# LUOJIUzxy/PortfolioOptGP

Hardware: AMD Instinct MI355X
Metric: GP fits/sec (N=4096, 1-D RBF) (higher is better)
Workload: dtype f64

## Files before the change

portfoliooptgp_amd/csrc/gpx_band16.hip:

```cpp
#include <hip/hip_runtime.h>
#include <hip/hip_ext.h>
#include "gpx_internal.h"
#include "gpx_leaf.h"
#include "gpx_b16core.h"

namespace gpx {


#ifdef GPX_BAND_PHASES
__device__ unsigned long long g_b16_phase[2][16];
#define Q_BEGIN unsigned long long qp_t = __builtin_amdgcn_s_memtime(), qp_acc[12] = {};
#define QP(i)                                                        \
  do {                                                               \
    const unsigned long long qp_n = __builtin_amdgcn_s_memtime();    \
    qp_acc[i] += qp_n - qp_t;                                        \
    qp_t = qp_n;                                                     \
  } while (0)
#define Q_END(kid)                                                                 \
  do {                                                                             \
    if (threadIdx.x == 0) {                                                        \
      for (int qp_i = 0; qp_i < 12; ++qp_i) atomicAdd(&g_b16_phase[kid][qp_i], qp_acc[qp_i]); \
      atomicAdd(&g_b16_phase[kid][15], 1ull);                                      \
    }                                                                              \
  } while (0)
#else
#define Q_BEGIN
#define QP(i) \
  do {        \
  } while (0)
#define Q_END(kid) \
  do {             \
  } while (0)
#endif

namespace {

__device__ __forceinline__ t4 ktile_t(const double* __restrict__ K, long long ld, int bi, int bj, int l15, int l4,
                                      int kband) {
  t4 t;
  const int gi = bi * 16 + l15;
#pragma unroll
  for (int r = 0; r < 4; ++r) {
    const int gj = bj * 16 + 4 * r + l4;
    const int i0 = max(gi, gj), j0 = min(gi, gj);
    const bool z = (i0 >> 6) - (j0 >> 6) >= kband;
    const double v = K[(long long)i0 * ld + (z ? i0 : j0)];
    t[r] = z ? 0.0 : v;
  }
  return t;
}

constexpr __host__ __device__ int wid(int i, int j) { return i * (i + 1) / 2 + j; }

__device__ __forceinline__ void exp4(const double (&x)[4], double (&e)[4]) {
  constexpr double c[13] = {0x1.71547652b82fep+0, -0x1.62e42fefa39efp-1, -0x1.abc9e3b39803fp-56,
                            0x1.ade156a5dcb37p-26, 0x1.28af3fca7ab0cp-22, 0x1.71dee623fde64p-19,
                            0x1.a01997c89e6b0p-16, 0x1.a01a014761f6ep-13, 0x1.6c16c1852b7b0p-10,
                            0x1.1111111122322p-7, 0x1.55555555502a1p-5, 0x1.5555555555511p-3,
                            0x1.000000000000bp-1};
  double k[4], r[4], p[4];
#pragma unroll
  for (int q = 0; q < 4; ++q) {
    k[q] = __builtin_rint(x[q] * c[0]);
    r[q] = __builtin_fma(k[q], c[1], x[q]);
  }
#pragma unroll
  for (int q = 0; q < 4; ++q) r[q] = __builtin_fma(k[q], c[2], r[q]);
#pragma unroll
  for (int q = 0; q < 4; ++q) p[q] = __builtin_fma(r[q], c[3], c[4]);
#pragma unroll
  for (int i = 5; i <= 12; ++i)
#pragma unroll
    for (int q = 0; q < 4; ++q) p[q] = __builtin_fma(r[q], p[q], c[i]);
#pragma unroll
  for (int q = 0; q < 4; ++q) {
    p[q] = __builtin_fma(r[q], p[q], 1.0);
    p[q] = __builtin_fma(r[q], p[q], 1.0);
    const double v = __builtin_amdgcn_ldexp(p[q], (int)k[q]);
    e[q] = !(x[q] < -1075.0) ? v : 0.0;
  }
}
struct ExpLib {
  __device__ __forceinline__ void load() {}
  __device__ __forceinline__ double exp(double x) const { return ::exp(x); }
  __device__ __forceinline__ void exp4(const double (&x)[4], double (&e)[4]) const { gpx::exp4(x, e); }
};

template <class EXP>
__device__ __forceinline__ double k_se1(double m2ai, double ai2, double aj, bool ok, bool diag, double var,
                                       double noise, const EXP& E) {
  if (!ok) return diag ? 1.0 : 0.0;
  const double v = var * E.exp(-0.5 * sqdist1_b(aj, m2ai, ai2));
  return diag ? v + noise : v;
}
__device__ __forceinline__ void ktile_store(double* __restrict__ K, long long ld, int bi, int bj, const t4& t, int l15,
                                            int l4) {
  double* p = K + (long long)(bi * 16 + l15) * ld + bj * 16 + l4;
#pragma unroll
  for (int r = 0; r < 4; ++r) p[4 * r] = t[r];
}
__device__ __forceinline__ int rq(int il) { return (il & 3) * 4 + (il >> 2); }

}

#ifndef GPX_B16_FWD3_WAVES
#define GPX_B16_FWD3_WAVES 2
#endif
template <int Q, bool KIN>
struct Fwd16 {
  static constexpr int kNew = 16 * kSC, kXa = kNew + (KIN ? 1 : Q + 1) * 256, size = kXa + (KIN ? Q + 1 : 1) * 16;
};
template <int Q, bool KIN>
__device__ __forceinline__ void fwd_sweep(const BandFusedArgs& a, double* __restrict__ lds) {
  double* sc = lds;
  double(*snew)[256] = reinterpret_cast<double(*)[256]>(lds + Fwd16<Q, KIN>::kNew);
  double(*sxa)[16] = reinterpret_cast<double(*)[16]>(lds + Fwd16<Q, KIN>::kXa);
  const unsigned long long wt0 = a.wtrace ? __builtin_amdgcn_s_memrealtime() : 0ull;
  const int b = a.active[blockIdx.x];
  const int Np = a.Np, nb = Np >> 4;
  const long long ld = a.ld;
  double* K = a.K + (long long)b * a.sMat;
  double* L = a.L + (long long)b * a.sMat;
  double* z = a.z + (long long)b * a.sVec;
  double* ldiag = a.ldiag + (long long)b * a.sVec;
  const bool kst = KIN && a.kstore;
  const double* y = a.Y + (long long)b * a.sY;
  const int n = a.nvalid[b];
  const int lane = threadIdx.x, l15 = lane & 15, l4 = lane >> 4;
  constexpr int NW = (Q + 1) * (Q + 2) / 2;
  const double* X = a.X + (long long)b * a.sX;
  int xd0 = 0;
  double kell = 1.0, kvar = 1.0, knoise = 0.0;
  ExpLib E;
  if constexpr (KIN) {
    E.load();
    const gpx_term& tm = a.specs[b].terms[0];
    const double* th = a.theta + (long long)b * GPX_THETA_STRIDE;
    xd0 = tm.dim_start;
    kell = th[tm.param_offset];
    kvar = th[tm.param_offset + 1];
    knoise = th[a.specs[b].n_params];
  }
  const int D = a.D;
  auto xval = [&](int g) { return X[(long long)min(g, n - 1) * D + xd0]; };
  t4 T[NW];
  double u[Q + 1];
  if constexpr (KIN) {
    if (l4 == 0) {
#pragma unroll
      for (int m = 0; m <= Q; ++m) sxa[m][rq(l15)] = m < nb ? xval(m * 16 + l15) / kell : 0.0;
    }
    wsync();
#pragma unroll
    for (int i = 0; i <= Q; ++i) {
      u[i] = 0.0;
      const double ar = i < nb ? xval(i * 16 + l15) / kell : 0.0;
      const int gi = i * 16 + l15;
#pragma unroll
      for (int j = 0; j <= i; ++j) {
        t4 t = tzero();
        if (i < nb) {
          const t4 ac = *reinterpret_cast<const t4*>(&sxa[j][4 * l4]);
#pragma unroll
          for (int r = 0; r < 4; ++r) {
            const int gj = j * 16 + 4 * r + l4;
            const bool zero = (gi >> 6) - (gj >> 6) >= a.kband;
            t[r] = zero ? 0.0 : k_se1(-2.0 * ar, ar * ar, ac[r], gi < n && gj < n, gi == gj, kvar, knoise, E);
          }
          if (kst) ktile_store(K, ld, i, j, t, l15, l4);
        }
        T[wid(i, j)] = t;
      }
    }
  } else {
#pragma unroll
    for (int i = 0; i <= Q; ++i) {
      u[i] = 0.0;
#pragma unroll
      for (int j = 0; j <= i; ++j) T[wid(i, j)] = (i < nb) ? ktile_t(K, ld, i, j, l15, l4, a.kband) : tzero();
    }
  }
  int gfail = 0;
  Q_BEGIN
  auto step = [&](const int k, const auto qkc, const auto fullc) __attribute__((always_inline)) {
    const int qk = qkc, k16 = k * 16;
    const int bn = k + Q + 1;
    const bool newrow = decltype(fullc)::value || bn < nb;
    double xn = 0.0;
    if constexpr (KIN) {
      if (newrow) xn = xval(bn * 16 + l15);
    } else {
      wsync();
      lds_drain();
      if (newrow) {
#pragma unroll
        for (int j = 0; j <= Q; ++j) tile_glds_swz(K + (long long)(bn * 16) * ld + (k + 1 + j) * 16, ld, snew[j], lane);
      }
    }
    double yl = y[min(k16 + l15, n - 1)];
    yl = k16 + l15 < n ? yl : 0.0;
    QP(0);
    t4 V;
    double lii;
    int fl;
    double* Lk = L + (long long)k * ((Q + 1) * 256);
    double zr[4];
    {
      t4 Wr;
      leaf16m(T[wid(0, 0)], V, Wr, lii, fl, sc, l15, l4);
      frag_store(Wr, Lk, lane);
      QP(1);
      const double yu = yl + u[0];
#pragma unroll
      for (int r = 0; r < 4; ++r) zr[r] = sum16(Wr[r] * yu);
    }
    if (fl >= 0 && gfail == 0) gfail = k16 + fl + 1;
    QP(2);
#pragma unroll
    for (int i = 1; i <= Q; ++i) {
      if (i <= qk) {
        t4 c = tzero();
        mma(c, V, T[wid(i, 0)]);
        T[wid(i, 0)] = c;
        double s = 0.0;
#pragma unroll
        for (int r = 0; r < 4; ++r) s = fma(c[r], zr[r], s);
        u[i] -= sum4(s);
      }
    }
    QP(3);
#pragma unroll
    for (int i = 1; i <= Q; ++i)
#pragma unroll
      for (int j = 1; j <= i; ++j)
        if (i <= qk) mms(T[wid(i, j)], T[wid(j, 0)], T[wid(i, 0)]);
    QP(4);
    vm_drain();
    wsync();
    QP(6);
#pragma unroll
    for (int i = 1; i <= Q; ++i)
      if (i <= qk) frag_store(T[wid(i, 0)], Lk + i * 256, lane);
    if (l4 == 0) ldiag[k16 + l15] = lii;
    if (l15 == 0) {
#pragma unroll
      for (int r = 0; r < 4; ++r) z[k16 + 4 * r + l4] = zr[r];
    }
#pragma unroll
    for (int i = 0; i < Q; ++i) {
#pragma unroll
      for (int j = 0; j <= i; ++j) T[wid(i, j)] = T[wid(i + 1, j + 1)];
      u[i] = u[i + 1];
    }
    u[Q] = 0.0;
    QP(7);
    if constexpr (KIN) {
      const double ar = xn / kell, m2ar = -2.0 * ar, ar2 = ar * ar;
      if (newrow && l4 == 0) sxa[bn % (Q + 1)][rq(l15)] = ar;
      wsync();
      const int gi = bn * 16 + l15;
#pragma unroll
      for (int j = 0; j <= Q; ++j) {
        t4 t = tzero();
        const int c = k + 1 + j;
        if (newrow && (bn >> 2) - (c >> 2) < a.kband) {
          const t4 ac = *reinterpret_cast<const t4*>(&sxa[c % (Q + 1)][4 * l4]);
          double xe[4], ev[4];
#pragma unroll
          for (int r = 0; r < 4; ++r) xe[r] = -0.5 * sqdist1_b(ac[r], m2ar, ar2);
          E.exp4(xe, ev);
          if (bn * 16 + 16 <= n) {
#pragma unroll
            for (int r = 0; r < 4; ++r) {
              const double v = kvar * ev[r];
              t[r] = (j == Q && 4 * r + l4 == l15) ? v + knoise : v;
            }
          } else {
#pragma unroll
            for (int r = 0; r < 4; ++r) {
              const int gj = c * 16 + 4 * r + l4;
              const double v = kvar * ev[r];
              t[r] = !(gi < n && gj < n) ? (gi == gj ? 1.0 : 0.0) : (gi == gj ? v + knoise : v);
            }
          }
          if (kst) ktile_store(K, ld, bn, c, t, l15, l4);
        }
        T[wid(Q, j)] = t;
      }
    } else {
#pragma unroll
      for (int j = 0; j <= Q; ++j) {
        t4 t = tzero();
        if (newrow) {
          const bool zero = (bn >> 2) - ((k + 1 + j) >> 2) >= a.kband;
#pragma unroll
          for (int r = 0; r < 4; ++r) {
            const int cl = 4 * r + l4;
            const double v = (j == Q && cl > l15) ? snew[j][swz16(cl, l15)] : snew[j][swz16(l15, cl)];
            t[r] = zero ? 0.0 : v;
          }
        }
        T[wid(Q, j)] = t;
      }
    }
    QP(5);
  };
  int k = 0;
  if constexpr (Q != 4)
    for (; k < nb - Q - 1; ++k) step(k, std::integral_constant<int, Q>{}, std::true_type{});
  for (; k < nb; ++k) step(k, min(Q, nb - 1 - k), std::false_type{});
  Q_END(0);
  if (lane == 0 && gfail > 0 && a.info[b] == 0) a.info[b] = gfail;
  wave_trace_put(a, wt0, Q);
}

template <int Q, bool KIN>
__global__ __launch_bounds__(64, Q <= 3 ? GPX_B16_FWD3_WAVES : (Q <= 4 ? 2 : 1)) void band16_fwd_kernel(BandFusedArgs a) {
  __shared__ __attribute__((aligned(16))) double lds[Fwd16<Q, KIN>::size];
  fwd_sweep<Q, KIN>(a, lds);
}

#ifndef GPX_B16_BWD_2W_QMAX
#define GPX_B16_BWD_2W_QMAX 3
#endif
template <int Q, int NT, bool SE1, bool KIN>
struct Bwd16 {
  static constexpr int kZ = 16 * kSC;
  static constexpr int nZ = SE1 ? (KIN ? 0 : 2 * (Q + 1)) : Q + 1;
  static constexpr int kAl = kZ + nZ * 256;
  static constexpr int kAlT = kAl + (SE1 ? 0 : (Q + 1) * 16);
  static constexpr int kXT = kAlT + (SE1 ? (Q + 1) * 16 : 0);
  static constexpr int kCs = kXT + (SE1 ? (Q + 1) * 16 : 0);
  static constexpr int kTh = kCs + (Q + 1) * 16;
  static constexpr int kRed = kTh + (SE1 ? 0 : 16);
  static constexpr bool LP = SE1 && KIN && Q == 4;
  static constexpr int kPf = kRed + (SE1 ? 0 : 16);
  static constexpr int size = kPf + (LP ? (Q + 1) * 256 : 0);
};
template <int Q, int NT, bool SE1, bool KIN>
__device__ __forceinline__ void bwd_sweep(const BandFusedArgs& a, double* __restrict__ lds, double* __restrict__ sx) {
  static_assert(!SE1 || KIN || Q <= 5, "the SE1 sweep double-buffers its K tiles in LDS: Q <= 5");
  static_assert(!KIN || SE1, "inline K tiles: SE1 sweeps only");
  using Ly = Bwd16<Q, NT, SE1, KIN>;
  double* sc = lds;
  double(*sz)[256] = reinterpret_cast<double(*)[256]>(lds + Ly::kZ);
  double(*sal)[16] = reinterpret_cast<double(*)[16]>(lds + Ly::kAl);
  double(*salT)[16] = reinterpret_cast<double(*)[16]>(lds + Ly::kAlT);
  double(*sxT)[16] = reinterpret_cast<double(*)[16]>(lds + Ly::kXT);
  double(*scs)[16] = reinterpret_cast<double(*)[16]>(lds + Ly::kCs);
  double* sth = SE1 ? lds : lds + Ly::kTh;
  double* sred = SE1 ? lds + 16 : lds + Ly::kRed;
  const unsigned long long wt0 = a.wtrace ? __builtin_amdgcn_s_memrealtime() : 0ull;
  const int b = a.active[blockIdx.x];
  const int Np = a.Np, nb = Np >> 4;
  const long long ld = a.ld;
  double* Kd = a.K + (long long)b * a.sMat;
  const double* L = a.L + (long long)b * a.sMat;
  const double* z = a.z + (long long)b * a.sVec;
  double* alpha = a.alpha + (long long)b * a.sVec;
  const double* X = a.X + (long long)b * a.sX;
  const int n = a.nvalid[b], D = a.D, nx = 16 * D;
  const int lane = threadIdx.x, l15 = lane & 15, l4 = lane >> 4;
  auto fetch = [&](int kk, double (&zr)[4], double (&xr)[2]) {
    const int q1 = min(Q, nb - 1 - kk), c16 = kk * 16;
    if constexpr (SE1 && !KIN) {
#pragma unroll
      for (int i = 0; i <= Q; ++i)
        if (i <= q1) tile_glds_swz(Kd + (long long)(c16 + 16 * i) * ld + c16, ld, sz[(kk & 1) * (Q + 1) + i], lane);
    }
#pragma unroll
    for (int r = 0; r < 4; ++r) zr[r] = z[c16 + 4 * r + l4];
#pragma unroll
    for (int h = 0; h < 2; ++h) {
      const int e = lane + 64 * h;
      xr[h] = X[min((long long)c16 * D + e, (long long)n * D - 1)];
    }
  };
  constexpr bool LP = Ly::LP;
  double* spf = lds + Ly::kPf;
  auto fetch_f = [&](int kk, t4& Wn, t4 (&Pn)[Q + 1]) {
    const int q1 = min(Q, nb - 1 - kk);
    const double* Lk = L + (long long)kk * ((Q + 1) * 256) + 4 * lane;
    if constexpr (LP) {
#pragma unroll
      for (int i = 0; i <= Q; ++i)
        if (i <= q1) {
          __builtin_amdgcn_global_load_lds(Lk + i * 256, spf + i * 256, 16, 0, 0);
          __builtin_amdgcn_global_load_lds(Lk + i * 256 + 2, spf + i * 256 + 128, 16, 0, 0);
        }
    } else {
      Wn = *reinterpret_cast<const t4*>(Lk);
#pragma unroll
      for (int i = 1; i <= Q; ++i) Pn[i] = (i <= q1) ? *reinterpret_cast<const t4*>(Lk + i * 256) : tzero();
    }
  };
  auto lds_tile = [&](int i) {
    const double2 a0 = *reinterpret_cast<const double2*>(spf + i * 256 + 2 * lane);
    const double2 a1 = *reinterpret_cast<const double2*>(spf + i * 256 + 128 + 2 * lane);
    return (t4){a0.x, a0.y, a1.x, a1.y};
  };
  double zr[4], xr[2];
  t4 Wn, Pn[Q + 1];
  fetch(nb - 1, zr, xr);
  fetch_f(nb - 1, Wn, Pn);
  {
    double* ldg = a.ldiag + (long long)b * a.sVec;
    for (int e = lane; e < Np; e += 64) ldg[e] = log(ldg[e]);
  }
  if (lane < GPX_THETA_STRIDE) sth[lane] = a.theta[b * GPX_THETA_STRIDE + lane];
  if (lane < 16) {
#pragma unroll
    for (int m = 0; m <= Q; ++m) {
      scs[m][lane] = 0.0;
      if constexpr (SE1) {
        salT[m][lane] = 0.0;
        sxT[m][lane] = 0.0;
      } else {
        sal[m][lane] = 0.0;
      }
    }
  }
  vm_drain();
  wsync();
  const DevSpec spec = a.specs[b];
  const int fkind = spec.terms[0].kind, fd0 = spec.terms[0].dim_start, fdn = spec.terms[0].dim_count;
  const bool fast = (NT == 1) && spec.n_terms == 1 && fkind >= GPX_SE && fkind <= GPX_EXPONENTIAL;
  const double fvar = sth[spec.terms[0].param_offset + 1];
  const double finv_ell = 1.0 / sth[spec.terms[0].param_offset];
  const double xscale = fast ? sth[spec.terms[0].param_offset] : 1.0;
  const double noise = sth[spec.n_params];
  double sums[NT][3];
#pragma unroll
  for (int t = 0; t < NT; ++t) sums[t][0] = sums[t][1] = sums[t][2] = 0.0;
  double snoise = 0.0, resmax = 0.0;
  constexpr int NS = Q * (Q + 1) / 2;
  t4 S[NS];
#pragma unroll
  for (int e = 0; e < NS; ++e) S[e] = tzero();
  double al[Q + 1];
  t4 R[Q + 1];
#pragma unroll
  for (int i = 0; i <= Q; ++i) {
    al[i] = 0.0;
    R[i] = tzero();
  }
  Q_BEGIN
  for (int k = nb - 1; k >= 0; --k) {
    const int qk = min(Q, nb - 1 - k), k16 = k * 16, cs = k % (Q + 1);
    t4 Wf, P[Q + 1];
    if constexpr (LP) {
      vm_drain();
      wsync();
      Wf = lds_tile(0);
#pragma unroll
      for (int i = 1; i <= Q; ++i) P[i] = (i <= qk) ? lds_tile(i) : tzero();
    } else {
      Wf = Wn;
#pragma unroll
      for (int i = 1; i <= Q; ++i) P[i] = Pn[i];
    }
    if constexpr (!SE1) {
#pragma unroll
      for (int h = 0; h < 2; ++h) {
        const int e = lane + 64 * h;
        if (e < nx) sx[cs * nx + e] = (k16 + e / D < n) ? xr[h] / xscale : 0.0;
      }
      for (int e = lane + 128; e < nx; e += 64) sx[cs * nx + e] = (k16 + e / D < n) ? X[(long long)k16 * D + e] / xscale : 0.0;
    } else {
#pragma unroll
      for (int h = 0; h < 2; ++h) {
        const int e = lane + 64 * h, il = e / D;
        if (e < nx && e - il * D == fd0) sxT[cs][(il & 3) * 4 + (il >> 2)] = (k16 + il < n) ? xr[h] / xscale : 0.0;
      }
    }
    const double zc[4] = {zr[0], zr[1], zr[2], zr[3]};
    lds_drain();
    wsync();
    if (k > 0) fetch(k - 1, zr, xr);
    QP(0);
    double t[4] = {0.0, 0.0, 0.0, 0.0};
#pragma unroll
    for (int i = 1; i <= Q; ++i) {
      double ai;
      if constexpr (LP)
        ai = salT[(k + i) % (Q + 1)][(l15 & 3) * 4 + (l15 >> 2)];
      else
        ai = al[i];
#pragma unroll
      for (int r = 0; r < 4; ++r) t[r] = fma(P[i][r], ai, t[r]);
    }
    double ap = 0.0;
#pragma unroll
    for (int r = 0; r < 4; ++r) ap = fma(Wf[r], zc[r] - sum16(t[r]), ap);
    ap = sum4(ap);
    al[0] = ap;
    if (l4 == 0) {
      if constexpr (SE1)
        salT[cs][(l15 & 3) * 4 + (l15 >> 2)] = ap;
      else
        sal[cs][l15] = ap;
    }
    QP(1);
#pragma unroll
    for (int i = 1; i <= Q; ++i) {
      t4 g = tzero();
      mma(g, P[i], Wf);
      P[i] = g;
    }
    QP(2);
    t4 Zn[Q + 1];
#pragma unroll
    for (int i = 1; i <= Q; ++i) {
      Zn[i] = tzero();
#pragma unroll
      for (int j = 1; j <= Q; ++j) {
        if (j >= i) {
          mms(Zn[i], S[wid(j - 1, i - 1)], P[j]);
        } else {
          const t4 tt = tile_transpose(S[wid(i - 1, j - 1)], sc, l15, l4);
          mms(Zn[i], tt, P[j]);
        }
      }
    }
    QP(3);
    if (k > 0) fetch_f(k - 1, Wn, Pn);
    t4 Zk = tzero();
    mma(Zk, Wf, Wf);
#pragma unroll
    for (int i = 1; i <= Q; ++i) mms(Zk, P[i], Zn[i]);
    wsync();
    QP(4);
    const int gj = k16 + l15;
    const bool jok = gj < n;
    const double* xj = sx + cs * nx + l15 * D;
    double colacc = 0.0;
    if constexpr (SE1) {
      const double xjv = sxT[cs][(l15 & 3) * 4 + (l15 >> 2)];
      const double m2xj = -2.0 * xjv, xj2 = xjv * xjv;
#pragma unroll
      for (int i = 0; i <= Q; ++i) {
        if (i > qk) continue;
        const t4& Zt = (i == 0) ? Zk : Zn[i];
        const int si = (k + i) % (Q + 1);
        const double w = i == 0 ? 1.0 : 2.0;
        const t4 a4 = *reinterpret_cast<const t4*>(&salT[si][4 * l4]);
        const t4 x4 = *reinterpret_cast<const t4*>(&sxT[si][4 * l4]);
        const bool zero = ((k + i) >> 2) - (k >> 2) >= a.kband;
        double r2v[4], kexp[4] = {0.0, 0.0, 0.0, 0.0};
#pragma unroll
        for (int r = 0; r < 4; ++r) r2v[r] = sqdist1_b(x4[r], m2xj, xj2);
        if constexpr (KIN) {
          if (!zero) {
            double xe[4];
#pragma unroll
            for (int r = 0; r < 4; ++r) xe[r] = -0.5 * r2v[r];
            exp4(xe, kexp);
          }
        }
#pragma unroll
        for (int r = 0; r < 4; ++r) {
          const int il = 4 * r + l4, gi = (k + i) * 16 + il;
          const double zij = Zt[r];
          const double ai = a4[r];
          const double r2 = r2v[r];
          const bool dg = i == 0 && il == l15;
          double kraw;
          if constexpr (KIN) {
            kraw = 0.0;
            if (!zero) {
              const double kv = fvar * kexp[r];
              kraw = dg ? kv + noise : kv;
            }
          } else {
            const bool up = i == 0 && il < l15;
            kraw = sz[(k & 1) * (Q + 1) + i][up ? swz16(l15, il) : swz16(il, l15)];
          }
          const double v = w * fma(ai, ap, -zij);
          const bool ok = i > 0 || (jok && gi < n);
          const double kij = KIN ? (ok ? kraw : 0.0) : ((zero || !ok) ? 0.0 : kraw);
          const double kg = i > 0 ? kij : (ok ? (dg ? fvar : kij) : 0.0);
          sums[0][0] = fma(v, kg * r2, sums[0][0]);
          sums[0][1] = fma(v, kg, sums[0][1]);
          snoise = (ok && dg) ? snoise + v : snoise;
          const double kz = kij * zij;
          colacc += kz;
          if (i > 0) R[i][r] += kz;
        }
      }
    } else {
#pragma unroll
      for (int i = 0; i <= Q; ++i)
        if (i <= qk) {
          const t4& Zt = (i == 0) ? Zk : Zn[i];
#pragma unroll
          for (int r = 0; r < 4; ++r) sz[i][(4 * r + l4) * 16 + l15] = Zt[r];
        }
      wsync();
      double rowp[Q + 1][4];
#pragma unroll
      for (int i = 0; i <= Q; ++i)
#pragma unroll
        for (int r = 0; r < 4; ++r) rowp[i][r] = 0.0;
      for (int i = 0; i <= qk; ++i) {
        const int si = (k + i) % (Q + 1);
        const double w = i == 0 ? 1.0 : 2.0;
#pragma unroll
        for (int r = 0; r < 4; ++r) {
          const int il = 4 * r + l4, gi = (k + i) * 16 + il;
          const double zij = sz[i][il * 16 + l15];
          const double ai = sal[si][il];
          const double* xi = sx + si * nx + il * D;
          const bool ok = jok && gi < n;
          const bool dg = i == 0 && gi == gj;
          const double v = w * fma(ai, ap, -zij);
          double kij = 0.0;
          if (ok) {
            double dk[NT][3];
            if (fast) {
              double d1[3];
              stationary_grad(fkind, sqdist_scaled(xi + fd0, xj + fd0, fdn), fvar, finv_ell, d1);
              dk[0][0] = d1[0]; dk[0][1] = d1[1]; dk[0][2] = d1[2];
              kij = fvar * d1[1];
            } else {
              kij = eval_k_grad<NT>(spec, sth, xi, xj, dk);
            }
#pragma unroll
            for (int q = 0; q < NT; ++q) {
              sums[q][0] = fma(v, dk[q][0], sums[q][0]);
              sums[q][1] = fma(v, dk[q][1], sums[q][1]);
              sums[q][2] = fma(v, dk[q][2], sums[q][2]);
            }
          }
          if (dg) kij += noise;
          snoise = (ok && dg) ? snoise + v : snoise;
          const double kz = ok ? kij * zij : 0.0;
          colacc += kz;
#pragma unroll
          for (int q = 1; q <= Q; ++q) rowp[q][r] = (q == i) ? kz : rowp[q][r];
        }
      }
#pragma unroll
      for (int i = 1; i <= Q; ++i)
#pragma unroll
        for (int r = 0; r < 4; ++r) R[i][r] += rowp[i][r];
    }
    QP(5);
    colacc = sum4(colacc);
    if (l4 == 0) scs[cs][l15] = colacc;
    auto finish = [&](int m, const t4& Rm) {
      const int sm = m % (Q + 1);
      wsync();
#pragma unroll
      for (int r = 0; r < 4; ++r) sc[(4 * r + l4) * kSC + l15] = Rm[r];
      wsync();
      if (lane < 16) {
        double rs = 0.0;
#pragma unroll
        for (int c = 0; c < 16; ++c) rs += sc[lane * kSC + c];
        const int g = m * 16 + lane;
        const double tot = scs[sm][lane] + rs;
        if (g < n) resmax = (tot == tot) ? fmax(resmax, fabs(tot - 1.0)) : INFINITY;
        scs[sm][lane] = 0.0;
      }
    };
    if (k + Q < nb) finish(k + Q, R[Q]);
    if (k == 0) {
#pragma unroll
      for (int m = Q - 1; m >= 0; --m)
        if (m < nb) finish(m, R[m]);
    }
    QP(7);
    vm_drain();
    wsync();
    QP(8);
    if (l4 == 0) alpha[k16 + l15] = ap;
#pragma unroll
    for (int r = 0; r < 4; ++r)
      if (4 * r + l4 == l15) Kd[(long long)(k16 + l15) * ld + k16 + l15] = Zk[r];
#pragma unroll
    for (int i = Q; i >= 2; --i) {
#pragma unroll
      for (int j = i; j >= 2; --j) S[wid(i - 1, j - 1)] = S[wid(i - 2, j - 2)];
      S[wid(i - 1, 0)] = Zn[i - 1];
    }
    S[wid(0, 0)] = Zk;
#pragma unroll
    for (int i = Q; i >= 1; --i) {
      if constexpr (!LP) al[i] = al[i - 1];
      R[i] = R[i - 1];
    }
    R[1] = tzero();
    QP(6);
  }
  Q_END(1);
  {
    double rm = (resmax == resmax) ? resmax : INFINITY;
#pragma unroll
    for (int o = 32; o >= 1; o >>= 1) rm = fmax(rm, __shfl_xor(rm, o, 64));
    if (lane == 0) a.results[(long long)b * kResStride + kResBandCheck] = rm;
  }
  double vals[GPX_MAX_TERMS * 3 + 1];
#pragma unroll
  for (int t = 0; t < GPX_MAX_TERMS; ++t)
#pragma unroll
    for (int q = 0; q < 3; ++q) vals[t * 3 + q] = t < NT ? wsum64(sums[t][q]) : 0.0;
  if (SE1) {
    vals[0] *= finv_ell;
    vals[1] /= fvar;
  }
  vals[GPX_MAX_TERMS * 3] = wsum64(snoise);
  if (lane == 0) {
#pragma unroll
    for (int v = 0; v < GPX_MAX_TERMS * 3 + 1; ++v) sred[v] = vals[v];
  }
  wsync();
  if (lane < GPX_THETA_STRIDE) {
    double* out = a.partial + (long long)b * a.sPartial;
    double s = 0.0;
    int slot = -1;
    const DevSpec* gs = a.specs + b;
    if (lane == gs->n_params) {
      slot = GPX_MAX_TERMS * 3;
    } else {
      for (int t = 0; t < gs->n_terms; ++t) {
        const int o = gs->terms[t].param_offset, kind = gs->terms[t].kind;
        const int np = (kind == GPX_RQ || kind == GPX_PERIODIC_SE) ? 3 : (kind == GPX_LINEAR ? 1 : 2);
        if (lane >= o && lane < o + np) slot = t * 3 + (lane - o);
      }
    }
    if (slot >= 0) s = sred[slot];
    out[lane] = s;
  }
  wave_trace_put(a, wt0, 16 + Q);
}

template <int Q, int NT, bool SE1, bool KIN>
__global__ __launch_bounds__(64, ((Q <= GPX_B16_BWD_2W_QMAX && SE1) || Bwd16<Q, NT, SE1, KIN>::LP) ? 2 : 1)
void band16_bwd_kernel(BandFusedArgs a) {
  extern __shared__ double sx[];
  __shared__ __attribute__((aligned(16))) double lds[Bwd16<Q, NT, SE1, KIN>::size];
  bwd_sweep<Q, NT, SE1, KIN>(a, lds, sx);
}

template <int Q, bool KIN_F, bool KIN_B>
__global__ __launch_bounds__(64, (Q <= GPX_B16_BWD_2W_QMAX) ? 2 : 1) void band16_fused_kernel(BandFusedArgs a) {
  constexpr int nf = Fwd16<Q, KIN_F>::size, nbk = Bwd16<Q, 1, true, KIN_B>::size;
  __shared__ __attribute__((aligned(16))) double lds[nf > nbk ? nf : nbk];
  fwd_sweep<Q, KIN_F>(a, lds);
  vm_drain();
  __threadfence();
  wsync();
  bwd_sweep<Q, 1, true, KIN_B>(a, lds, nullptr);
}

constexpr int kB16Tiles = 16;
__global__ __launch_bounds__(256) void band16_build_kernel(BuildArgs a, int Q) {
  const int b = a.active[blockIdx.y];
  const int nb = a.rows >> 4, ntiles = nb * (Q + 1);
  const int lane = threadIdx.x & 63;
  const int t0 = (blockIdx.x * 4 + (threadIdx.x >> 6)) * kB16Tiles;
  if (t0 >= ntiles) return;
  const int n = a.nvalid[b], D = a.D;
  const double* X = a.X + (long long)b * a.sX;
  const double* th = a.theta + (long long)b * GPX_THETA_STRIDE;
  const DevSpec& spec = a.specs[b];
  const int k0 = spec.terms[0].kind;
  const bool fast = spec.n_terms == 1 && k0 >= GPX_SE && k0 <= GPX_EXPONENTIAL;
  const double noise = th[spec.n_params];
  const gpx_term& tm = spec.terms[0];
  const double ell = th[tm.param_offset], var = th[tm.param_offset + 1];
  const int d0 = tm.dim_start, dn = tm.dim_count;
  for (int t = t0; t < min(t0 + kB16Tiles, ntiles); ++t) {
    const int m = t / (Q + 1), d = t - m * (Q + 1);
    if (m < d) continue;
    const int gi = m * 16 + (lane >> 2), gj0 = (m - d) * 16 + (lane & 3) * 4;
    double* out = a.out + (long long)b * a.sOut + (long long)gi * a.ldo + gj0;
    double v[4];
    if (fast) {
      const double* xi = X + (long long)min(gi, n - 1) * D + d0;
      const double xi0 = gi < n ? xi[0] / ell : 0.0;
#pragma unroll
      for (int q = 0; q < 4; ++q) {
        const int gj = gj0 + q;
        if (gi < n && gj < n) {
          const double* xj = X + (long long)gj * D + d0;
          const double r2 = dn == 1 ? sqdist1(xi0, xj[0] / ell) : sqdist_gpflow(xi, xj, dn, ell);
          switch (k0) {
            case GPX_SE: v[q] = stationary_value<GPX_SE>(r2, var); break;
            case GPX_MATERN12: v[q] = stationary_value<GPX_MATERN12>(r2, var); break;
            case GPX_MATERN32: v[q] = stationary_value<GPX_MATERN32>(r2, var); break;
            case GPX_MATERN52: v[q] = stationary_value<GPX_MATERN52>(r2, var); break;
            default: v[q] = stationary_value<GPX_EXPONENTIAL>(r2, var); break;
          }
          if (gi == gj) v[q] += noise;
        } else {
          v[q] = gi == gj ? 1.0 : 0.0;
        }
      }
    } else {
      const DevSpec sp = spec;
#pragma unroll
      for (int q = 0; q < 4; ++q) {
        const int gj = gj0 + q;
        if (gi < n && gj < n) {
          v[q] = eval_k(sp, th, X + (long long)gi * D, X + (long long)gj * D);
          if (gi == gj) v[q] += noise;
        } else {
          v[q] = gi == gj ? 1.0 : 0.0;
        }
      }
    }
#pragma unroll
    for (int q = 0; q < 4; ++q) out[q] = v[q];
  }
}

__global__ __launch_bounds__(64) void slow_gather_kernel(const int* __restrict__ act, int n,
                                                          const double* __restrict__ res, int stride,
                                                          double* __restrict__ out, const int* __restrict__ info,
                                                          int* __restrict__ info_out) {
  const int t = blockIdx.x * 64 + threadIdx.x;
  if (t >= n * stride) return;
  const int i = t / stride, c = t - i * stride, b = act[i];
  out[t] = res[(long long)b * stride + c];
  if (c == 0) info_out[i] = info[b];
  __threadfence_system();
}

__global__ __launch_bounds__(64) void slow_inputs_kernel(const int* __restrict__ act, int n, int* __restrict__ act_out,
                                                         const double* __restrict__ theta, double* __restrict__ theta_out,
                                                         const int* __restrict__ bandp, int* __restrict__ bandp_out,
                                                         int* __restrict__ info_out, int B, int r0, int r1) {
  const int t = blockIdx.x * 64 + threadIdx.x;
  if (t < B * GPX_THETA_STRIDE) theta_out[t] = theta[t];
  if (t < n) act_out[t] = (t >= r0 && t < r1) ? act[r0 + r1 - 1 - t] : act[t];
  if (t < B) {
    bandp_out[t] = bandp[t];
    info_out[t] = 0;
  }
}

void launch_slow_inputs(const int* act, int n, int* act_out, const double* theta, double* theta_out, const int* bandp,
                        int* bandp_out, int* info_out, int B, hipStream_t s, int r0, int r1) {
  const int m = std::max(B * GPX_THETA_STRIDE, n);
  hipLaunchKernelGGL(slow_inputs_kernel, dim3((m + 63) / 64), dim3(64), 0, s, act, n, act_out, theta, theta_out, bandp,
                     bandp_out, info_out, B, r0, r1);
}

void launch_slow_gather(const int* act, int n, const double* res, int stride, double* out, const int* info,
                        int* info_out, hipStream_t s) {
  if (n <= 0) return;
  hipLaunchKernelGGL(slow_gather_kernel, dim3((n * stride + 63) / 64), dim3(64), 0, s, act, n, res, stride, out,
                     info, info_out);
}

__global__ __launch_bounds__(64) void spin_us_kernel(int us) {
  const unsigned long long t0 = __builtin_amdgcn_s_memrealtime();
  while (__builtin_amdgcn_s_memrealtime() - t0 < 100ull * (unsigned long long)us) {
  }
}
void launch_spin_us(int us, hipStream_t s) { hipLaunchKernelGGL(spin_us_kernel, dim3(1), dim3(64), 0, s, us); }

__global__ __launch_bounds__(64) void wave_marker_kernel(BandFusedArgs a, int kind) {
  wave_trace_put(a, __builtin_amdgcn_s_memrealtime(), kind);
}

void launch_wave_marker(unsigned long long* wt, unsigned int* wn, unsigned int cap, int kind, hipStream_t s) {
  BandFusedArgs a{};
  a.wtrace = wt;
  a.wtrace_n = wn;
  a.wtrace_cap = cap;
  hipLaunchKernelGGL(wave_marker_kernel, dim3(1), dim3(64), 0, s, a, kind);
}

void launch_band16_build(const BuildArgs& a, int Q, int n_active, hipStream_t s) {
  const int tiles = (a.rows >> 4) * (Q + 1), per_wg = 4 * kB16Tiles;
  hipLaunchKernelGGL(band16_build_kernel, dim3((tiles + per_wg - 1) / per_wg, n_active), dim3(256), 0, s, a, Q);
}

template <int Q, bool KF, bool KB>
__device__ __forceinline__ void fused_sweeps(const BandFusedArgs& a, double* __restrict__ lds) {
  fwd_sweep<Q, KF>(a, lds);
  vm_drain();
  __threadfence();
  wsync();
  bwd_sweep<Q, 1, true, KB>(a, lds, nullptr);
}
template <int Q, bool KF, bool KB>
constexpr int fused_lds() {
  return Fwd16<Q, KF>::size > Bwd16<Q, 1, true, KB>::size ? Fwd16<Q, KF>::size : Bwd16<Q, 1, true, KB>::size;
}
template <bool KF, bool KB, int WQ>
__global__ __launch_bounds__(64, 1) void band16_wide_kernel(BandFusedArgs a) {
  constexpr int n4 = fused_lds<4, KF, KB>(), n5 = fused_lds<5, KF, KB>();
  constexpr int n8 = WQ > 5 ? fused_lds<8, KF, KB>() : 0;
  constexpr int n45 = n4 > n5 ? n4 : n5;
  __shared__ __attribute__((aligned(16))) double lds[n45 > n8 ? n45 : n8];
  const int Q = a.bandp[a.active[blockIdx.x]];
  if constexpr (WQ > 5) {
    if (Q == 8) return fused_sweeps<8, KF, KB>(a, lds);
    if (Q == 7) return fused_sweeps<7, KF, KB>(a, lds);
    if (Q == 6) return fused_sweeps<6, KF, KB>(a, lds);
  }
  if (Q == 5)
    fused_sweeps<5, KF, KB>(a, lds);
  else
    fused_sweeps<4, KF, KB>(a, lds);
}

void launch_band16_wide(const BandFusedArgs& a, int kin, int n_active, hipStream_t s, hipEvent_t* ev, int wq) {
  auto k = (kin & 1) ? ((kin & 2) ? (wq > 5 ? band16_wide_kernel<true, true, 8> : band16_wide_kernel<true, true, 5>)
                                  : band16_wide_kernel<true, false, 5>)
                     : ((kin & 2) ? band16_wide_kernel<false, true, 5> : band16_wide_kernel<false, false, 5>);
  if (ev) {
    hipExtLaunchKernelGGL(k, dim3(n_active), dim3(64), 0, s, ev[0], ev[1], 0, a);
    (void)hipEventRecord(ev[2], s);
    (void)hipEventRecord(ev[3], s);
    return;
  }
  hipLaunchKernelGGL(k, dim3(n_active), dim3(64), 0, s, a);
}

template <int Q>
static void launch16_q(const BandFusedArgs& a, int max_terms, bool se1, int kin, int n_active, hipStream_t s,
                       hipEvent_t* ev) {
  kin = se1 ? kin : 0;
  static const bool fused = [] {
    const char* e = getenv("GPX_B16_FUSED");
    return e && atoi(e) != 0;
  }();
  if (se1 && fused) {
    auto fk = (kin & 1) ? ((kin & 2) ? band16_fused_kernel<Q, true, true> : band16_fused_kernel<Q, true, false>)
                        : ((kin & 2) ? band16_fused_kernel<Q, false, true> : band16_fused_kernel<Q, false, false>);
    if (ev) {
      hipExtLaunchKernelGGL(fk, dim3(n_active), dim3(64), 0, s, ev[0], ev[1], 0, a);
      (void)hipEventRecord(ev[2], s);
      (void)hipEventRecord(ev[3], s);
      return;
    }
    hipLaunchKernelGGL(fk, dim3(n_active), dim3(64), 0, s, a);
    return;
  }
  auto fwd = (kin & 1) ? band16_fwd_kernel<Q, true> : band16_fwd_kernel<Q, false>;
  auto bwd = se1 ? ((kin & 2) ? band16_bwd_kernel<Q, 1, true, true> : band16_bwd_kernel<Q, 1, true, false>)
                 : max_terms <= 1 ? band16_bwd_kernel<Q, 1, false, false>
                                  : max_terms == 2 ? band16_bwd_kernel<Q, 2, false, false>
                                                   : band16_bwd_kernel<Q, GPX_MAX_TERMS, false, false>;
  const size_t xs = se1 ? 0 : (size_t)(Q + 1) * 16 * a.D * sizeof(double);
  if (ev) {
    hipExtLaunchKernelGGL(fwd, dim3(n_active), dim3(64), 0, s, ev[0], ev[1], 0, a);
    hipExtLaunchKernelGGL(bwd, dim3(n_active), dim3(64), xs, s, ev[2], ev[3], 0, a);
    return;
  }
  hipLaunchKernelGGL(fwd, dim3(n_active), dim3(64), 0, s, a);
  hipLaunchKernelGGL(bwd, dim3(n_active), dim3(64), xs, s, a);
}

template <int Q>
static void launch16_wide_q(const BandFusedArgs& a, int n_active, hipStream_t s, hipEvent_t* ev) {
  auto fwd = band16_fwd_kernel<Q, true>;
  auto bwd = band16_bwd_kernel<Q, 1, true, true>;
  if (ev) {
    hipExtLaunchKernelGGL(fwd, dim3(n_active), dim3(64), 0, s, ev[0], ev[1], 0, a);
    hipExtLaunchKernelGGL(bwd, dim3(n_active), dim3(64), 0, s, ev[2], ev[3], 0, a);
    return;
  }
  hipLaunchKernelGGL(fwd, dim3(n_active), dim3(64), 0, s, a);
  hipLaunchKernelGGL(bwd, dim3(n_active), dim3(64), 0, s, a);
}

void launch_band16(const BandFusedArgs& a, int Q, int max_terms, bool se1, int kin, int n_active, hipStream_t s,
                   hipEvent_t* ev) {
  switch (Q) {
    case 1: launch16_q<1>(a, max_terms, se1, kin, n_active, s, ev); break;
    case 2: launch16_q<2>(a, max_terms, se1, kin, n_active, s, ev); break;
    case 3: launch16_q<3>(a, max_terms, se1, kin, n_active, s, ev); break;
    case 4: launch16_q<4>(a, max_terms, se1, kin, n_active, s, ev); break;
    case 5: launch16_q<5>(a, max_terms, se1, kin, n_active, s, ev); break;
    case 6: launch16_wide_q<6>(a, n_active, s, ev); break;
    case 7: launch16_wide_q<7>(a, n_active, s, ev); break;
    default: launch16_wide_q<8>(a, n_active, s, ev); break;
  }
}

}

#ifdef GPX_BAND_PHASES
extern "C" int gpx_debug_band16_phases(unsigned long long* out, int reset) {
  if (hipMemcpyFromSymbol(out, HIP_SYMBOL(gpx::g_b16_phase), sizeof(gpx::g_b16_phase)) != hipSuccess) return -1;
  if (reset) {
    static const unsigned long long zero[2][16] = {};
    if (hipMemcpyToSymbol(HIP_SYMBOL(gpx::g_b16_phase), zero, sizeof(zero)) != hipSuccess) return -1;
  }
  return 0;
}
#endif
```

Before: 19390.

## Spill outer band-window tile rows to LDS rings for wide Q sweeps

For wide bands (Q>=7 with kernel-in-kernel), the forward and backward band Cholesky sweeps now keep their last one or two rows of 16x16 tiles in LDS ring buffers instead of registers. The backward sweep also moves its residual accumulators to an LDS ring. The goal is to cut VGPR pressure and avoid scratch spills in the Q=7/8 paths. In exchange it adds LDS traffic, extra wave syncs and a larger shared allocation. It only affects wide-band cases, which may not be used at N=4096 with a 1-D RBF kernel.

```diff
diff --git a/portfoliooptgp_amd/csrc/gpx_band16.hip b/portfoliooptgp_amd/csrc/gpx_band16.hip
--- a/portfoliooptgp_amd/csrc/gpx_band16.hip
+++ b/portfoliooptgp_amd/csrc/gpx_band16.hip
@@ -106,9 +106,19 @@
 #ifndef GPX_B16_FWD3_WAVES
 #define GPX_B16_FWD3_WAVES 2
 #endif
+#ifndef GPX_B16_FWD7_LDS_ROWS
+#define GPX_B16_FWD7_LDS_ROWS 1
+#endif
+#ifndef GPX_B16_FWD8_LDS_ROWS
+#define GPX_B16_FWD8_LDS_ROWS 2
+#endif
 template <int Q, bool KIN>
 struct Fwd16 {
-  static constexpr int kNew = 16 * kSC, kXa = kNew + (KIN ? 1 : Q + 1) * 256, size = kXa + (KIN ? Q + 1 : 1) * 16;
+  static constexpr int NL = !KIN ? 0 : (Q >= 8 ? GPX_B16_FWD8_LDS_ROWS : (Q == 7 ? GPX_B16_FWD7_LDS_ROWS : 0));
+  static constexpr int QR = Q - NL;
+  static constexpr bool LW = NL > 0;
+  static constexpr int kNew = 16 * kSC, kXa = kNew + (KIN ? (LW ? 0 : 1) : Q + 1) * 256, kRing = kXa + (KIN ? Q + 1 : 1) * 16;
+  static constexpr int size = kRing + NL * (Q + 1) * 256;
 };
 template <int Q, bool KIN>
 __device__ __forceinline__ void fwd_sweep(const BandFusedArgs& a, double* __restrict__ lds) {
@@ -127,7 +137,14 @@
   const double* y = a.Y + (long long)b * a.sY;
   const int n = a.nvalid[b];
   const int lane = threadIdx.x, l15 = lane & 15, l4 = lane >> 4;
-  constexpr int NW = (Q + 1) * (Q + 2) / 2;
+  using Ly = Fwd16<Q, KIN>;
+  constexpr bool LW = Ly::LW;
+  constexpr int QR = Ly::QR;
+  constexpr int NW = (QR + 1) * (QR + 2) / 2;
+  auto ring = [&](int R, int C) __attribute__((always_inline)) {
+    constexpr int nl = LW ? Ly::NL : 1;
+    return reinterpret_cast<t4*>(lds + Ly::kRing + ((R % nl) * (Q + 1) + C % (Q + 1)) * 256 + 4 * lane);
+  };
   const double* X = a.X + (long long)b * a.sX;
   int xd0 = 0;
   double kell = 1.0, kvar = 1.0, knoise = 0.0;
@@ -169,7 +186,10 @@
           }
           if (kst) ktile_store(K, ld, i, j, t, l15, l4);
         }
-        T[wid(i, j)] = t;
+        if (!LW || i <= QR)
+          T[wid(i, j)] = t;
+        else
+          *ring(i, j) = t;
       }
     }
   } else {
@@ -220,8 +240,14 @@
     for (int i = 1; i <= Q; ++i) {
       if (i <= qk) {
         t4 c = tzero();
-        mma(c, V, T[wid(i, 0)]);
-        T[wid(i, 0)] = c;
+        if (!LW || i <= QR) {
+          mma(c, V, T[wid(i, 0)]);
+          T[wid(i, 0)] = c;
+        } else {
+          t4* p = ring(k + i, k);
+          mma(c, V, *p);
+          *p = c;
+        }
         double s = 0.0;
 #pragma unroll
         for (int r = 0; r < 4; ++r) s = fma(c[r], zr[r], s);
@@ -233,14 +259,39 @@
     for (int i = 1; i <= Q; ++i)
 #pragma unroll
       for (int j = 1; j <= i; ++j)
-        if (i <= qk) mms(T[wid(i, j)], T[wid(j, 0)], T[wid(i, 0)]);
+        if (i <= qk && (!LW || i <= QR)) mms(T[wid(i, j)], T[wid(j, 0)], T[wid(i, 0)]);
+    if constexpr (LW) {
+#pragma unroll
+      for (int i = QR + 1; i <= Q; ++i) {
+        if (i <= qk) {
+          const t4 pi = *ring(k + i, k);
+#pragma unroll
+          for (int j = 1; j <= i; ++j) {
+            t4* p = ring(k + i, k + j);
+            t4 t = *p;
+            if (j <= QR)
+              mms(t, T[wid(j <= QR ? j : 0, 0)], pi);
+            else if (j < i)
+              mms(t, *ring(k + j, k), pi);
+            else
+              mms(t, pi, pi);
+            *p = t;
+          }
+        }
+      }
+    }
     QP(4);
     vm_drain();
     wsync();
     QP(6);
 #pragma unroll
     for (int i = 1; i <= Q; ++i)
-      if (i <= qk) frag_store(T[wid(i, 0)], Lk + i * 256, lane);
+      if (i <= qk) {
+        if (!LW || i <= QR)
+          frag_store(T[wid(i, 0)], Lk + i * 256, lane);
+        else
+          frag_store(*ring(k + i, k), Lk + i * 256, lane);
+      }
     if (l4 == 0) ldiag[k16 + l15] = lii;
     if (l15 == 0) {
 #pragma unroll
@@ -249,10 +300,16 @@
 #pragma unroll
     for (int i = 0; i < Q; ++i) {
 #pragma unroll
-      for (int j = 0; j <= i; ++j) T[wid(i, j)] = T[wid(i + 1, j + 1)];
+      for (int j = 0; j <= i; ++j) {
+        if (!LW || i < QR)
+          T[wid(i, j)] = T[wid(i + 1, j + 1)];
+        else if (i == QR)
+          T[wid(i, j)] = *ring(k + i + 1, k + j + 1);
+      }
       u[i] = u[i + 1];
     }
     u[Q] = 0.0;
+    if constexpr (LW) wsync();
     QP(7);
     if constexpr (KIN) {
       const double ar = xn / kell, m2ar = -2.0 * ar, ar2 = ar * ar;
@@ -285,7 +342,10 @@
           }
           if (kst) ktile_store(K, ld, bn, c, t, l15, l4);
         }
-        T[wid(Q, j)] = t;
+        if constexpr (LW)
+          *ring(bn, c) = t;
+        else
+          T[wid(Q, j)] = t;
       }
     } else {
 #pragma unroll
@@ -322,6 +382,12 @@
 
 #ifndef GPX_B16_BWD_2W_QMAX
 #define GPX_B16_BWD_2W_QMAX 3
+#endif
+#ifndef GPX_B16_BWD7_LDS_ROWS
+#define GPX_B16_BWD7_LDS_ROWS 0
+#endif
+#ifndef GPX_B16_BWD8_LDS_ROWS
+#define GPX_B16_BWD8_LDS_ROWS 2
 #endif
 template <int Q, int NT, bool SE1, bool KIN>
 struct Bwd16 {
@@ -333,9 +399,14 @@
   static constexpr int kCs = kXT + (SE1 ? (Q + 1) * 16 : 0);
   static constexpr int kTh = kCs + (Q + 1) * 16;
   static constexpr int kRed = kTh + (SE1 ? 0 : 16);
-  static constexpr bool LP = SE1 && KIN && Q == 4;
+  static constexpr bool LP = SE1 && KIN && (Q == 4 || Q >= 7);
   static constexpr int kPf = kRed + (SE1 ? 0 : 16);
-  static constexpr int size = kPf + (LP ? (Q + 1) * 256 : 0);
+  static constexpr bool LW = SE1 && KIN && Q >= 7;
+  static constexpr int NLB = !LW ? 0 : (Q >= 8 ? GPX_B16_BWD8_LDS_ROWS : GPX_B16_BWD7_LDS_ROWS);
+  static constexpr int QRB = Q - NLB;
+  static constexpr int kRr = kPf + (LP ? (Q + 1) * 256 : 0);
+  static constexpr int kSr = kRr + (LW ? Q * 256 : 0);
+  static constexpr int size = kSr + NLB * Q * 256;
 };
 template <int Q, int NT, bool SE1, bool KIN>
 __device__ __forceinline__ void bwd_sweep(const BandFusedArgs& a, double* __restrict__ lds, double* __restrict__ sx) {
@@ -399,6 +470,16 @@
     const double2 a1 = *reinterpret_cast<const double2*>(spf + i * 256 + 128 + 2 * lane);
     return (t4){a0.x, a0.y, a1.x, a1.y};
   };
+  constexpr bool LW = Ly::LW;
+  constexpr int NLB = Ly::NLB, QRB = Ly::QRB;
+  static_assert(QRB >= 1, "at least one window row stays in registers");
+  auto rring = [&](int m) __attribute__((always_inline)) {
+    return reinterpret_cast<t4*>(lds + Ly::kRr + (m % Q) * 256 + 4 * lane);
+  };
+  auto sring = [&](int R, int C) __attribute__((always_inline)) {
+    constexpr int nl = NLB > 0 ? NLB : 1;
+    return lds + Ly::kSr + ((R % nl) * Q + C % Q) * 256;
+  };
   double zr[4], xr[2];
   t4 Wn, Pn[Q + 1];
   fetch(nb - 1, zr, xr);
@@ -419,6 +500,9 @@
         sal[m][lane] = 0.0;
       }
     }
+  }
+  if constexpr (LW) {
+    for (int e = 0; e < Q + NLB * Q; ++e) *reinterpret_cast<t4*>(lds + Ly::kRr + e * 256 + 4 * lane) = tzero();
   }
   vm_drain();
   wsync();
@@ -433,7 +517,7 @@
 #pragma unroll
   for (int t = 0; t < NT; ++t) sums[t][0] = sums[t][1] = sums[t][2] = 0.0;
   double snoise = 0.0, resmax = 0.0;
-  constexpr int NS = Q * (Q + 1) / 2;
+  constexpr int NS = QRB * (QRB + 1) / 2;
   t4 S[NS];
 #pragma unroll
   for (int e = 0; e < NS; ++e) S[e] = tzero();
@@ -514,7 +598,17 @@
       Zn[i] = tzero();
 #pragma unroll
       for (int j = 1; j <= Q; ++j) {
-        if (j >= i) {
+        if (LW && (j >= i ? j : i) > QRB) {
+          t4 x;
+          if (j >= i) {
+            x = *reinterpret_cast<const t4*>(sring(k + j, k + i) + 4 * lane);
+          } else {
+            const double* p = sring(k + i, k + j) + 64 * (l15 & 3) + 4 * l4 + (l15 >> 2);
+#pragma unroll
+            for (int r = 0; r < 4; ++r) x[r] = p[16 * r];
+          }
+          mms(Zn[i], x, P[j]);
+        } else if (j >= i) {
           mms(Zn[i], S[wid(j - 1, i - 1)], P[j]);
         } else {
           const t4 tt = tile_transpose(S[wid(i - 1, j - 1)], sc, l15, l4);
@@ -547,6 +641,9 @@
         const t4 x4 = *reinterpret_cast<const t4*>(&sxT[si][4 * l4]);
         const bool zero = ((k + i) >> 2) - (k >> 2) >= a.kband;
         double r2v[4], kexp[4] = {0.0, 0.0, 0.0, 0.0};
+        t4 rr = tzero();
+        if constexpr (LW)
+          if (i > 0) rr = *rring(k + i);
 #pragma unroll
         for (int r = 0; r < 4; ++r) r2v[r] = sqdist1_b(x4[r], m2xj, xj2);
         if constexpr (KIN) {
@@ -584,8 +681,14 @@
           snoise = (ok && dg) ? snoise + v : snoise;
           const double kz = kij * zij;
           colacc += kz;
-          if (i > 0) R[i][r] += kz;
-        }
+          if constexpr (LW) {
+            if (i > 0) rr[r] += kz;
+          } else {
+            if (i > 0) R[i][r] += kz;
+          }
+        }
+        if constexpr (LW)
+          if (i > 0) *rring(k + i) = rr;
       }
     } else {
 #pragma unroll
@@ -663,11 +766,21 @@
         scs[sm][lane] = 0.0;
       }
     };
-    if (k + Q < nb) finish(k + Q, R[Q]);
-    if (k == 0) {
-#pragma unroll
-      for (int m = Q - 1; m >= 0; --m)
-        if (m < nb) finish(m, R[m]);
+    if constexpr (LW) {
+      if (k + Q < nb) finish(k + Q, *rring(k + Q));
+      *rring(k) = tzero();
+      if (k == 0) {
+#pragma unroll
+        for (int m = Q - 1; m >= 0; --m)
+          if (m < nb) finish(m, m > 0 ? *rring(m) : tzero());
+      }
+    } else {
+      if (k + Q < nb) finish(k + Q, R[Q]);
+      if (k == 0) {
+#pragma unroll
+        for (int m = Q - 1; m >= 0; --m)
+          if (m < nb) finish(m, R[m]);
+      }
     }
     QP(7);
     vm_drain();
@@ -677,19 +790,28 @@
 #pragma unroll
     for (int r = 0; r < 4; ++r)
       if (4 * r + l4 == l15) Kd[(long long)(k16 + l15) * ld + k16 + l15] = Zk[r];
-#pragma unroll
-    for (int i = Q; i >= 2; --i) {
+    if constexpr (NLB > 0) {
+#pragma unroll
+      for (int i = QRB; i <= Q - 1; ++i) *reinterpret_cast<t4*>(sring(k + i, k) + 4 * lane) = Zn[i];
+#pragma unroll
+      for (int j = 1; j <= QRB; ++j) *reinterpret_cast<t4*>(sring(k + QRB, k + j) + 4 * lane) = S[wid(QRB - 1, j - 1)];
+      wsync();
+    }
+#pragma unroll
+    for (int i = QRB; i >= 2; --i) {
 #pragma unroll
       for (int j = i; j >= 2; --j) S[wid(i - 1, j - 1)] = S[wid(i - 2, j - 2)];
       S[wid(i - 1, 0)] = Zn[i - 1];
     }
     S[wid(0, 0)] = Zk;
-#pragma unroll
-    for (int i = Q; i >= 1; --i) {
-      if constexpr (!LP) al[i] = al[i - 1];
-      R[i] = R[i - 1];
-    }
-    R[1] = tzero();
+    if constexpr (!LW) {
+#pragma unroll
+      for (int i = Q; i >= 1; --i) {
+        if constexpr (!LP) al[i] = al[i - 1];
+        R[i] = R[i - 1];
+      }
+      R[1] = tzero();
+    }
     QP(6);
   }
   Q_END(1);
@@ -735,7 +857,7 @@
 }
 
 template <int Q, int NT, bool SE1, bool KIN>
-__global__ __launch_bounds__(64, ((Q <= GPX_B16_BWD_2W_QMAX && SE1) || Bwd16<Q, NT, SE1, KIN>::LP) ? 2 : 1)
+__global__ __launch_bounds__(64, ((Q <= GPX_B16_BWD_2W_QMAX && SE1) || (Bwd16<Q, NT, SE1, KIN>::LP && Q <= 4)) ? 2 : 1)
 void band16_bwd_kernel(BandFusedArgs a) {
   extern __shared__ double sx[];
   __shared__ __attribute__((aligned(16))) double lds[Bwd16<Q, NT, SE1, KIN>::size];
@@ -893,7 +1015,8 @@
 template <bool KF, bool KB, int WQ>
 __global__ __launch_bounds__(64, 1) void band16_wide_kernel(BandFusedArgs a) {
   constexpr int n4 = fused_lds<4, KF, KB>(), n5 = fused_lds<5, KF, KB>();
-  constexpr int n8 = WQ > 5 ? fused_lds<8, KF, KB>() : 0;
+  constexpr int n67 = fused_lds<6, KF, KB>() > fused_lds<7, KF, KB>() ? fused_lds<6, KF, KB>() : fused_lds<7, KF, KB>();
+  constexpr int n8 = WQ > 5 ? (n67 > fused_lds<8, KF, KB>() ? n67 : fused_lds<8, KF, KB>()) : 0;
   constexpr int n45 = n4 > n5 ? n4 : n5;
   __shared__ __attribute__((aligned(16))) double lds[n45 > n8 ? n45 : n8];
   const int Q = a.bandp[a.active[blockIdx.x]];
```

Result: slower. 18880 (-2.6%).
